# l646773422/h264-lab

Measured on AMD Instinct MI355X. Metric: 1080p macroblocks/sec, higher is better.
Workload: dtype u8

## Files before the change

h264-lab_amd/csrc/enc_mb.h:

```cpp
#ifndef H264E_ENC_MB_H
#define H264E_ENC_MB_H

#include <stddef.h>
#include "enc_kernels.h"

struct GCtx { mv32 mv_left[4], mv_tl[4], mv_top[8]; };
#define GSCR_OFF(t) ((t) == 0 ? 0 : (t) == 1 ? 1024 : (t) == 2 ? 1536 : 2048)
#define GSCR_BYTES 2304

struct MbBuf
{
    alignas(16) uint8_t inp[256];
    alignas(16) uint8_t inp_c[128];
    alignas(16) uint8_t pred[256];
    alignas(4) uint8_t pix_top[36];
    alignas(4) uint8_t ptop[96];
    mv32 mv_top[8];
    uint8_t nnz_top[8];
    int8_t i4_top[4];
    uint32_t df_nz_top;
    int top_type, top_qp;
    mv32 mv[16], mvd[16];
    int type, cost, used_cand;
    mv32 mv_skip_pred;
// ... 309 lines not shown
                    const uint32_t q00 = IP(mv), q02 = IP(v02), q20 = IP(v20), q22 = IP(v22);
#undef IP
                    probe(r, q00, q02, q20, q22);
                }
            }
            sv[0] = (int)t0; sv[1] = (int)t1; sv[2] = (int)t2; sv[3] = (int)t3; sv[4] = (int)t4; sv[5] = (int)t5; sv[6] = (int)t6;
        }, s8);
        wave_sync();
        int best = -1, c8[8];
        mv32 vbest = mv;
        {
            const int pax = hp_pq_vertical, p_step = pax ? mvy(pq) : mvx(pq), s_step = pax ? mvx(sq) : mvy(sq);
            const int p_mv = pax ? mvy(mv) : mvx(mv), s_mv = pax ? mvx(mv) : mvy(mv), p_pr = pax ? mvy(mv_pred) : mvx(mv_pred), s_pr = pax ? mvx(mv_pred) : mvy(mv_pred);
            int P[4], S[4];
            grp_eval4([&](int k) -> int { return se_len((int16_t)(p_mv + k*p_step) - p_pr); }, P);
            grp_eval4([&](int k) -> int { return se_len((int16_t)(s_mv + k*s_step) - s_pr); }, S);
            c8[0] = MUL_LAMBDA(P[2] + S[0], m.lambda_mv); c8[1] = MUL_LAMBDA(P[1] + S[0], m.lambda_mv); c8[2] = MUL_LAMBDA(P[0] + S[2], m.lambda_mv);
            c8[3] = MUL_LAMBDA(P[0] + S[1], m.lambda_mv); c8[4] = MUL_LAMBDA(P[1] + S[1], m.lambda_mv); c8[5] = MUL_LAMBDA(P[2] + S[2], m.lambda_mv);
            c8[6] = MUL_LAMBDA(P[2] + S[1], m.lambda_mv);
        }
#define TRY(j, vv) { const int cst = s8[j] + c8[j]; if (cst < min_sad) { min_sad = cst; vbest = (vv); best = j; } }
        TRY(0, v02) TRY(1, v01) TRY(2, v20) TRY(3, v10) TRY(4, v11) TRY(5, v22) TRY(6, v12)
#undef TRY
        const int pa = best < 0 ? 0 : best == 0 ? 1 : best == 1 ? 0 : best == 2 ? 2 : best == 3 ? 0 : best == 4 ? 1 : best == 5 ? 3 : 3;
        const int pb = best == 1 ? 1 : best == 3 ? 2 : best == 4 ? 2 : best == 6 ? 1 : pa;
        GRP_FOR(i)
        {
            for (int k = 0; k < npass; k++)
            {
                const int d = i + 16*k, r = d >> (g >> 1), c4 = d & (g - 1), o = w*r + 4*c4;
                const uint32_t x = lds32(scr + pa*plane + o), y = lds32(scr + pb*plane + o);
                lds32_store(dst + 16*r + 4*c4, AVG4(x, y));
            }
        }
#undef AVG4
        wave_sync();
        mv = vbest;
    }
    STAMP(L, 26);
    return min_sad;
}

DEV void search_type(RowLds &L, const MbBuf &B, const MbCtx &m, int t, mv32 mv_best, int sad_best0, const rect_t &lim, int skip_cost)
{
    GCtx &X = L.gctx[t];
    int imv = 0, part_sad = MUL_LAMBDA(t == 0 ? 1 : t == 3 ? 12 : 4, m.lambda_q4);
    const int w = (t & 2) ? 8 : 16, h = (t & 1) ? 8 : 16;
    int px = 0, py = 0;
    uint8_t *test = L.gtest[t], *scr = L.gscr + GSCR_OFF(t);
    for (;;)
    {
        rect_t range;
        mv32 mvabs = mb_abs(m, mv_best);
        int sad_best = sad_best0;
        const mv32 mvp = mvp_get_arr(X.mv_left, X.mv_tl, X.mv_top, m.avail, px >> 2, py >> 2, w >> 2, h >> 2);
        if (!t) set_range(mvabs, range, lim, m.y*64 + py*4);
        else
        {
            mvabs = mvround(mb_abs(m, mvp));
            set_range(mvabs, range, lim, m.y*64 + py*4);
            sad_best = grp_sad_ref(m.rv, px + (mvx(mvabs) >> 2), py + (mvy(mvabs) >> 2), B.inp + 16*py + px, w, h)
                     + mv_cost(m, mvabs, mb_abs(m, mvp));
        }
        STAMP(L, 24);
        part_sad += diamond_g(L, B, m, px, py, mvabs, range, mb_abs(m, mvp), sad_best, w, h, test + 16*py + px, scr);
        const mv32 mv = mvsub(mvabs, mvmk(m.x*64, m.y*64));
        L.part_mvd[t][imv] = mvsub(mv, mvp);
        L.part_mv[t][imv++] = mv;
        mvp_put_arr(X.mv_left, X.mv_tl, X.mv_top, px >> 2, py >> 2, w >> 2, h >> 2, mv);
        wave_sync();
        STAMP(L, 27);
        if (t == 0) L.early_bound = imax(part_sad, skip_cost);
        px = (px + w) & 15;
        if (!px)
        {
            py = (py + h) & 15;
            if (!py) break;
        }
    }
    L.gcost[t] = part_sad;
    L.gnum[t] = imv;
}

DEV void partition_hints(const int sad[4], int mode[4])
{
    int sum = sad[0] + sad[1] + sad[2] + sad[3];
    int slope = iabs((sad[0] - sad[2]) + (sad[1] - sad[3])) - iabs((sad[0] - sad[1]) + (sad[2] - sad[3]));
    int skew = iabs(sad[3] - sad[0]) - iabs(sad[2] - sad[1]);
    if (slope > (sum >> 4)) mode[1] = 1;
    if (slope < -(sum >> 4)) mode[2] = 1;
    if (iabs(skew) > (sum >> 4) && iabs(slope) <= (sum >> 4)) mode[3] = 1;
}

DEV void predict_chroma_inter(const MbBuf &B, const MbCtx &m, uint8_t *pred_c)
{
    int w = (m.type & 2) ? 4 : 8, h = (m.type & 1) ? 4 : 8, part = 0, x = 0, y = 0;
    if (m.type == -1) w = h = 8;
    for (;; part++)
    {
        wave_interp_chroma(m.rv, m.ref[1], m.ref[2], x, y, mb_abs(m, B.mv[part]), w, h, pred_c + 16*y + x);
        x = (x + w) & 7;
        if (!x)
        {
            y = (y + h) & 7;
            if (!y) break;
        }
    }
}

DEV int skip_chroma_ok(const MbBuf &B, const MbCtx &m, const uint8_t *pred_c)
{
    const int thr = m.skip_thr;
    for (int c = 0; c < 2; c++)
    {
        int sad = wave_sum([&](int l) -> int {
            if (l >= 16) return 0;
            int r = l >> 1, g = l & 1;
            uint32_t a = lds32(B.inp_c + 16*r + 8*c + 4*g);
            uint32_t p = (m.cropped && r < 4) ? lds32(B.inp_c + 16*(2*r + c) + 8*c + 4*g) : lds32(pred_c + 16*r + 8*c + 4*g);
            return (int)sad4_u8(a, p, 0);
        });
        if (sad >= thr) return 0;
    }
    return 1;
}

template <class SIG> DEV void inter_choose(RowLds &L, MbBuf &B, MbCtx &m, SIG sig)
{
    int prefer[4] = { 1, 0, 0, 0 };
    const RefView &R = m.rv;
    const int bx = m.x*16, by = m.y*16;
    int sad, sad_skip = 0x7FFFFFFF, sad_best = 0x7FFFFFFF, cand_cost_best = 0, j = 0, ncand = 0, sad4[4];
    mv32 mv_best = MV_NA;
    LaneArr cand;
    cand.clear();

    const mv32 mv_pred16 = mvp_get(L, B, m, 0, 0, 4, 4);
    m.mv_skip_pred = 0;
    if (!(~m.avail & (AV_L | AV_T)) && L.mv_left[0] != 0 && B.mv_top[0] != 0) m.mv_skip_pred = mv_pred16;
    const mv32 mv_skip = m.mv_skip_pred, mv_skip_a = mb_abs(m, mv_skip);

    STAMP(L, 2);
    if (in_rect(mv_skip_a, mv_qlimit(m)))
    {
        wave_interp_luma(R, 0, 0, mv_skip_a, 16, 16, L.skip_pred);
        sad_skip = wave_sad_lds_q(B.inp, L.skip_pred, sad4);
        if (imax(imax(sad4[0], sad4[1]), imax(sad4[2], sad4[3])) < m.skip_thr)
        {
            m.type = -1;
            B.mv[0] = mv_skip;
            m.cost = 0;
            predict_chroma_inter(B, m, L.skip_pred_c);
            if (skip_chroma_ok(B, m, L.skip_pred_c))
            {
                wave_copy_wh(B.pred, L.skip_pred, 16, 16);
                return;
            }
        }
        if (m.speed < 1) partition_hints(sad4, prefer);
        mv_best = mvround(mv_skip);
        cand.set(ncand++, mv_best);
        if (!((mvx(mv_skip) | mvy(mv_skip)) & 3))
        {
            sad_best = sad_skip;
            cand_cost_best = mv_cost(m, mv_skip, mv_pred16);
            j = 1;
// ... 453 lines not shown
```

h264-lab_amd/csrc/enc_selftest.h:

```cpp
#ifndef H264E_ENC_SELFTEST_H
#define H264E_ENC_SELFTEST_H
#include "enc_row.h"

struct StageLds
{
    alignas(16) uint8_t win[WIN_W*WIN_STRIDE + 16];
    alignas(16) uint8_t a[256], b[256], o[256];
    alignas(16) qblk_t q[16];
    alignas(4) int16_t dc[16], lev[16], coef[16];
    alignas(4) uint16_t qdat[42];
    CavlcTab ct;
    I4Scratch i4s;
    DfTab df;
    alignas(16) uint8_t yt[20*YT_STRIDE];
    alignas(16) uint8_t ctile[2][10*CT_STRIDE];
    alignas(4) uint8_t bs[32];
    alignas(4) uint8_t nb[5*24];
};
#define STAGE_IN_MAX (96*96 + 256)
#define STAGE_NARGS 24
#define STAGE_OUT_MAX (16 + 16*64 + 32 + 32 + 256)
DEV void stage_selftest(StageLds &S, RowLds &L, int stage, const GLOBAL_AS uint8_t *in, const int *args, GLOBAL_AS uint8_t *out)
{
    int a[STAGE_NARGS];
// ... 40 lines not shown
            if (l < 8) { lds32_store((uint8_t *)S.dc + 4*l, 0u); lds32_store((uint8_t *)S.lev + 4*l, 0u); }
            for (int k = l; k < 256; k += 64) lds32_store((uint8_t *)S.q + 4*k, 0u);
        }
        wave_sync();
        unsigned nz = 0;
        int dcflag = 0;
        WAVE_FOR(l) { lds32_store(S.o + 4*l, lds32(S.b + 4*l)); }
        wave_sync();
        if (mode == QMODE_INTER) nz = wave_xform_quant_recon<QMODE_INTER>(S.a, S.b, S.o, 16, S.q, S.dc, S.lev, S.qdat, (int *)0);
        else if (mode == QMODE_I16) nz = wave_xform_quant_recon<QMODE_I16>(S.a, S.b, S.o, 16, S.q, S.dc, S.lev, S.qdat, (int *)0);
        else if (mode == QMODE_CHROMA) nz = wave_xform_quant_recon<QMODE_CHROMA>(S.a, S.b, S.o, 16, S.q, S.dc, S.lev, S.qdat, &dcflag);
        else nz = i4_block_code(i4q_make(S.qdat), S.a, S.b, S.o, 16, S.q);
        wave_sync();
        WAVE_FOR(l)
        {
            for (int k = l; k < 256; k += 64) gstore32((gu8 *)out + 8 + 4*k, lds32((const uint8_t *)S.q + 4*k));
            if (l < 8) { gstore32((gu8 *)out + 8 + 1024 + 4*l, lds32((const uint8_t *)S.dc + 4*l)); gstore32((gu8 *)out + 8 + 1056 + 4*l, lds32((const uint8_t *)S.lev + 4*l)); }
        }
        wave_sync();
        WAVE_FOR(l) { gstore32((gu8 *)out + 8 + 1088 + 4*l, lds32(S.o + 4*l)); }
        if (wave_lane() == 0) { oi[0] = (int32_t)nz; oi[1] = dcflag; }
        (void)side;
    } else if (stage == 5)
    {
        cavlc_tab_load(S.ct);
        WAVE_FOR(l) { if (l < 8) lds32_store((uint8_t *)S.coef + 4*l, gload32((const gu8 *)in + 4*l)); }
        wave_sync();
        BitW b;
        b.acc = 0; b.nacc = 0; b.pos = 0; b.cap = 60; b.overflow = 0; b.buf = (GLOBAL_AS uint32_t *)(out + 8);
        const int nnz = cavlc_block(b, S.ct, S.coef, a[0], a[1], a[2]);
        const uint32_t nbits = bw_bits(b);
        if (b.nacc) bw_put(b, 32 - b.nacc, 0);
        if (wave_lane() == 0) { oi[0] = nnz; oi[1] = (int32_t)nbits; }
    } else if (stage == 6)
    {
        WAVE_FOR(l)
        {
            if (l < 13)
            {
                const uint8_t e = in[l];
                if (l < 4) S.nb[24*(4 - l) + 3] = e;
                else S.nb[3 + (l - 4)] = e;
            }
            if (l < 16) lds32_store(S.a + 4*l, gload32((const gu8 *)in + 16 + 4*l));
            if (l < 16) lds32_store(S.o + 4*l, 0u);
        }
        wave_sync();
        const int res = wave_i4_choose(S.a, S.o, a[0], S.nb + 24 + 4, a[1], a[2], S.i4s, i4_lanes_make(24));
        wave_sync();
        WAVE_FOR(l) { if (l < 16) gstore32((gu8 *)out + 8 + 4*l, lds32(S.o + 4*l)); }
        if (wave_lane() == 0) { oi[0] = res & 15; oi[1] = res >> 4; }
    } else if (stage == 7)
    {
        const int ny = 20*YT_STRIDE, nc = 10*CT_STRIDE;
        df_tab_load(S.df);
        WAVE_FOR(l)
        {
            for (int k = l; k < ny; k += 64) S.yt[k] = in[k];
            for (int k = l; k < nc; k += 64) { S.ctile[0][k] = in[ny + k]; S.ctile[1][k] = in[ny + nc + k]; }
            if (l < 32) S.bs[l] = in[ny + 2*nc + l];
        }
        wave_sync();
        wave_deblock(S.yt, S.ctile[0], S.ctile[1], S.bs, a[0], a[1], a[2], S.df);
        wave_sync();
        WAVE_FOR(l)
        {
            for (int k = l; k < ny; k += 64) out[k] = S.yt[k];
            for (int k = l; k < nc; k += 64) { out[ny + k] = S.ctile[0][k]; out[ny + nc + k] = S.ctile[1][k]; }
        }
    } else if (stage == 8)
    {
        h264e_geom_t Gs;
        MbCtx m;
        Plane P8 = { (const gu8 *)in, 96, 96, 96 };
        Gs.width = Gs.W = 96; Gs.height = Gs.H = 96; Gs.nmbx = Gs.nmby = 6; Gs.nmb = 36; Gs.cropping = 0;
        Gs.lim_x0 = a[15]; Gs.lim_y0 = a[16]; Gs.lim_x1 = a[17]; Gs.lim_y1 = a[18];
        m.G = &Gs; m.speed = a[10]; m.slice_type = 0; m.x = 2; m.y = 2; m.num = 14; m.qp = a[9];
        m.lambda_mv = k_lambda_mv_q4[a[9]];
        m.rv = R; m.rv.P = P8; m.rv.nmbx = 6; m.rv.nmby = 6;
        if (a[19]) { m.rv.has_win = 1; m.rv.win = (const lu8 *)L.win; m.rv.wx0 = 32 - WIN_M; m.rv.wy0 = 32 - WIN_M; wave_load_window(L.win, P8, m.rv.wx0, m.rv.wy0, 0); }
        WAVE_FOR(l) { lds32_store(L.mb[0].inp + 4*l, gload32((const gu8 *)in + 96*96 + 4*l)); lds32_store(L.gtest[0] + 4*l, 0u); }
        wave_sync();
        const rect_t range = { a[11], a[12], a[13], a[14] };
        GRP_EACH(grp)
        {
            if (grp == (a[20] & 3))
            {
                mv32 mv = mvmk(a[4], a[5]);
                const int cost = diamond_g(L, L.mb[0], m, a[0], a[1], mv, range, mvmk(a[6], a[7]), a[8], a[2], a[3], L.gtest[0] + 16*a[1] + a[0], L.gscr);
                L.gcost[0] = cost; L.gcost[1] = mvx(mv); L.gcost[2] = mvy(mv);
            }
        }
        wave_sync();
        WAVE_FOR(l) { gstore32((gu8 *)out + 16 + 4*l, lds32(L.gtest[0] + 4*l)); }
        if (wave_lane() == 0) { oi[0] = L.gcost[0]; oi[1] = L.gcost[1]; oi[2] = L.gcost[2]; }
    }
}

DEV uint32_t sv_h32(uint32_t a)
{
    a ^= a >> 16; a *= 0x7feb352du; a ^= a >> 15; a *= 0x846ca68bu; a ^= a >> 16;
    return a;
}
DEV int sv_lattice(int32_t ix, int32_t iy, uint32_t seed) { return (int)(sv_h32((uint32_t)ix*0x9E3779B1u ^ (uint32_t)iy*0x85EBCA77u ^ seed) & 255); }
DEV int sv_tex(int32_t X, int32_t Y, uint32_t seed, int lg)
{
    int32_t c = 1 << lg, ix = X >> lg, iy = Y >> lg, fx = X & (c - 1), fy = Y & (c - 1);
    int32_t a = sv_lattice(ix, iy, seed), b = sv_lattice(ix + 1, iy, seed), cc = sv_lattice(ix, iy + 1, seed), d = sv_lattice(ix + 1, iy + 1, seed);
    int32_t top = a*(c - fx) + b*fx, bot = cc*(c - fx) + d*fx;
    return (top*(c - fy) + bot*fy + (1 << (2*lg - 1))) >> (2*lg);
}
DEV uint8_t sv_sample(int w, int h, int t, uint32_t seed, int idx)
{
    const int32_t OFF = 1 << 20;
    if (idx < w*h)
    {
        int x = idx % w, y = idx / w, fw = w/8 > 32 ? w/8 : 32, fh = h/6 > 32 ? h/6 : 32;
        int fx0 = (w/2 + ((10*t) >> 2)) % (w - fw), fy0 = h/3, v;
        if (x >= fx0 && x < fx0 + fw && y >= fy0 && y < fy0 + fh) v = sv_tex(4*x - 10*t + OFF, 4*y + OFF, seed + 1, 5);
        else v = (sv_tex(4*x + 5*t + OFF, 4*y + 3*t + OFF, seed, 6)*3 >> 2) + 32;
        v += (int)(sv_h32((uint32_t)x ^ ((uint32_t)y << 12) ^ ((uint32_t)t << 24) ^ (uint32_t)(seed*7919u)) % 5) - 2;
        return (uint8_t)clip255(v);
    }
    idx -= w*h;
    const int cw = w/2, ch = h/2, pl = idx >= cw*ch;
    if (pl) idx -= cw*ch;
    int x = idx % cw, y = idx / cw;
    if (!pl) return (uint8_t)(128 + ((sv_tex(8*x + 5*t + OFF, 8*y + 3*t + OFF, seed + 2, 7) - 128) >> 2));
    return (uint8_t)(128 - ((sv_tex(8*x + 5*t + OFF, 8*y + 3*t + OFF, seed + 3, 7) - 128) >> 3));
}

#endif
```

h264-lab_amd/csrc/h264e_kernels.hip:

```cpp
#include <stdio.h>
#include <stdlib.h>
#include <string.h>
#include "enc_row.h"
#include "enc_selftest.h"
#include "../../include/h264e_hip.h"

#include <hip/hip_runtime.h>





#ifndef H264E_POLL_SLEEP
#define H264E_POLL_SLEEP 16
#endif
DEV int poll_progress(const GLOBAL_AS int *flag, int need, int &seen, unsigned spin_limit)
{
    unsigned spins = 0;
    for (;;)
    {
        seen = uni(__hip_atomic_load(flag, __ATOMIC_RELAXED, __HIP_MEMORY_SCOPE_AGENT));
        if (seen >= need) return 0;
        if (seen < 0) return seen;
        if (++spins > spin_limit) return -1;
// ... 300 lines not shown
                }
                seen_dep = lowest;
                if (!st) consumer_acquire();
            }
            STAMP(L, 13);
            if (WAVES >= 2 && !st && x >= 2) st = lds_wait(&L.f_wdone, x - 1, &L.f_stop);
            STAMP(L, 23);
            if (!st) row_prefetch<GEOM>(L, G, RT, row, x);
            STAMP(L, 0);
            if (uni(abort_v) == launch_id) st = -2;
            if (!st && seen < need)
            {
                seen = uni(early);
                if (seen < 0) st = seen;
                else if (seen < need) st = poll_progress(above, need, seen, G.spin_limit);
                if (!st) consumer_acquire();
            }
            STAMP(L, 13);
            if (!st) load_top<WAVES >= 2 ? LOAD_TOP_MV : LOAD_TOP_ALL>(L, L.mb[x & 1], G, C.bottom + (size_t)(row - 1)*G.nmbx, C.pend + (size_t)(row - 1)*G.nmbx, x, row > row0);
            STAMP(L, 0);
            if (WAVES >= 2 && !st && x >= 1) st = lds_wait(&L.f_decided, x, &L.f_stop);
            STAMP(L, 6);
            if (st)
            {
                if (WAVES >= 2) { flag_set(&L.f_stop, st); return; }
                if (LANE == 0)
                {
                    if (st == -1) *errflag = 1;
                    __hip_atomic_store(my_progress, st, __ATOMIC_RELAXED, __HIP_MEMORY_SCOPE_AGENT);
                }
                count_mbs(x);
                return;
            }
            if (WAVES == 1) row_step<GEOM>(L, G, C, RT, row, x, row0, row1);
            else mb_search<GEOM>(L, L.mb[x & 1], G, RT, row, x, row0, SearchSignals{ &L, x + 1, WAVES >= 3 });
            if (WAVES >= 3 && uni(flag_get(&L.f_stop))) return;
            {
                const int ff = uni(L.far_fail[0]) | (WAVES == 1 ? uni(L.far_fail[1]) : 0);
                if (ff)
                {
                    if (WAVES >= 2) { flag_set(&L.f_stop, ff < -2 ? -2 : ff); return; }
                    if (LANE == 0)
                    {
                        if (ff == -1) *errflag = 1;
                        __hip_atomic_store(my_progress, ff < -2 ? -2 : ff, __ATOMIC_RELAXED, __HIP_MEMORY_SCOPE_AGENT);
                    }
                    count_mbs(x);
                    return;
                }
            }
            if (WAVES >= 2) { flag_set(&L.f_inter, x + 1); STAMP(L, 14); continue; }
            asm volatile("s_waitcnt vmcnt(0)" ::: "memory");
            __builtin_amdgcn_wave_barrier();
            publish(my_progress, x + 1);
            STAMP(L, 14);
        }
        if (WAVES >= 2)
        {
#ifdef H264E_STAMPS
            if (LANE < 32 && C.prof) atomicAdd(C.prof + LANE, L.prof[0][LANE]);
#endif
            return;
        }
    } else if (WAVES >= 3 && wv == 2)
    {
        for (int x = 0; x < G.nmbx; x++)
        {
            int req = 0, st = 0;
            for (unsigned spins = 0;; spins++)
            {
                const int r3 = uni(flag_get(&L.f_t3req));
                if (r3 == x + 1) { req = 1; break; }
                if (r3 > x + 1) break;
                if (uni(flag_get(&L.f_inter)) >= x + 1) break;
                if (uni(flag_get(&L.f_stop))) { st = 1; break; }
                if (spins > LDS_SPIN_LIMIT) { flag_set(&L.f_stop, -1); st = 1; break; }
                __builtin_amdgcn_s_sleep(H264E_LDS_SLEEP);
            }
            if (st) return;
            if (!req) continue;
            MbCtx m;
            mb_ctx_init<GEOM>(m, L, G, RT, row, x, row0, 2);
            const rect_t lim = { uni(L.t3_lim[0]), uni(L.t3_lim[1]), uni(L.t3_lim[2]), uni(L.t3_lim[3]) };
            const mv32 mv_best = (mv32)uni(L.t3_mv_best);
            const int sad_best = uni(L.t3_sad_best);
            GRP_EACH(t)
            {
                if (t == 3) search_type(L, L.mb[x & 1], m, 3, mv_best, sad_best, lim, 0);
            }
            wave_sync();
            const int ff = uni(L.far_fail[2]);
            if (ff) { flag_set(&L.f_stop, ff < -2 ? -2 : ff); return; }
            flag_set(&L.f_t3done, x + 1);
        }
#ifdef H264E_STAMPS
        if (LANE < 32 && C.prof) atomicAdd(C.prof + LANE, L.prof[2][LANE]);
#endif
        return;
    } else if (WAVES == 4 && wv == 3)
    {
        for (int x = 0; x < G.nmbx; x++)
        {
            const int st = lds_wait(&L.f_front, x + 1, &L.f_stop);
            if (st)
            {
                if (LANE == 0) __hip_atomic_store(my_progress, st == -2 ? -2 : -1, __ATOMIC_RELAXED, __HIP_MEMORY_SCOPE_AGENT);
                return;
            }
            MbCtx m;
            mb_ctx_init<GEOM>(m, L, G, RT, row, x, row0, 1);
            m.type = uni(L.d_type[x & 1]);
            mb_recon_back<GEOM>(L, L.mb[x & 1], m, G, C, RT, row, x, row0, row1);
            asm volatile("s_waitcnt vmcnt(0)" ::: "memory");
            __builtin_amdgcn_wave_barrier();
            publish(my_progress, x + 1);
            flag_set(&L.f_wdone, x + 1);
        }
#ifdef H264E_STAMPS
        if (LANE < 32 && C.prof) atomicAdd(C.prof + LANE, L.prof[3][LANE]);
#endif
        return;
    } else
    {
        GLOBAL_AS int *my_decided = my_progress + G.nmby;
        GLOBAL_AS h264e_mbbottom_t *rowrec = C.bottom + (size_t)row*G.nmbx;
        int seen = 0;
        for (int x = 0; x < G.nmbx; x++)
        {
            MbBuf &B = L.mb[x & 1];
            MbCtx m;
            mb_ctx_init<GEOM>(m, L, G, RT, row, x, row0, 1);
            int ff = 0;
            const int need = row > row0 ? imin(x + 2, G.nmbx) : 0;
            if (seen < need)
            {
                ff = poll_progress(C.progress + (row - 1), need, seen, G.spin_limit);
                if (!ff) consumer_acquire();
                else flag_set(&L.f_stop, ff);
            }
            STAMP(L, 17);
            if (!ff)
            {
                load_top<LOAD_TOP_REST>(L, B, G, C.bottom + (size_t)(row - 1)*G.nmbx, C.pend + (size_t)(row - 1)*G.nmbx, x, row > row0);
                if (!mb_intra_decide(L, B, m, RT, InterFromSearchWave{ &L, x + 1, WAVES == 4 })) ff = uni(flag_get(&L.f_stop));
                else
                {
                    flag_set(&L.f_decided, x + 1);
                    WAVE_FOR(l) { if (l < 4) cstore32((gu8 *)(rowrec + x) + 32 + 4*l, (uint32_t)B.mv_top[l]); }
                    const auto publish_decided = [&]() {
                        asm volatile("s_waitcnt vmcnt(0)" ::: "memory");
                        __builtin_amdgcn_wave_barrier();
                        publish(my_decided, x + 1);
                    };
                    if (WAVES == 4)
                    {
                        mb_recon_front<GEOM>(L, B, m, G, C, RT, row, x, row0, row1, publish_decided);
                        L.d_type[x & 1] = m.type;
                    } else mb_recon_write<GEOM>(L, B, m, G, C, RT, row, x, row0, row1, publish_decided);
                    ff = uni(L.far_fail[1]);
                    if (ff) { ff = ff < -2 ? -2 : ff; flag_set(&L.f_stop, ff); }
                    else if (WAVES == 4) flag_set(&L.f_front, x + 1);
                }
            }
            if (ff)
            {
                if (LANE == 0)
                {
                    if (ff == -1) *errflag = 1;
                    __hip_atomic_store(my_decided, ff, __ATOMIC_RELAXED, __HIP_MEMORY_SCOPE_AGENT);
                    if (WAVES != 4) __hip_atomic_store(my_progress, ff, __ATOMIC_RELAXED, __HIP_MEMORY_SCOPE_AGENT);
                }
                count_mbs(x);
                return;
// ... 101 lines not shown
```

h264-lab_amd/csrc/wave.h:

```cpp
#ifndef H264E_WAVE_H
#define H264E_WAVE_H

#include <stdint.h>
#include <string.h>

#ifdef H264E_EMU
extern "C" void emu_check_global(const void *p, size_t n, const char *file, int line);
#define EMU_GLOBAL(p, n) emu_check_global((const void *)(p), (n), __FILE__, __LINE__)
#define GLOBAL_AS
#define LDS_AS
#define NOINLINE_DEV static __attribute__((noinline))
#define DEV static inline
#define DEVM inline
#define DCONST static const
#ifdef H264E_EMU_REVERSE
#define WAVE_FOR(l) for (int l = 63; l >= 0; --l)
#else
#define WAVE_FOR(l) for (int l = 0; l < 64; ++l)
#endif
struct u32x4 { uint32_t x, y, z, w; };
DEV void wave_sync() {}
DEV int wave_lane() { return 0; }
DEV int uni(int v) { return v; }
template <class F> DEV int wave_sum(F f)
{
    int s = 0;
    for (int l = 0; l < 64; ++l) s += f(l);
    return s;
}
template <class F> DEV void wave_sum4(F f, int out[4])
{
    out[0] = out[1] = out[2] = out[3] = 0;
    for (int l = 0; l < 64; ++l)
    {
        int v[4] = { 0, 0, 0, 0 };
        f(l, v);
        for (int k = 0; k < 4; ++k) out[k] += v[k];
    }
}
template <class F> DEV void wave_sum8(F f, int out[8])
{
    for (int k = 0; k < 8; ++k) out[k] = 0;
    for (int l = 0; l < 64; ++l)
    {
        int v[8] = { 0, 0, 0, 0, 0, 0, 0, 0 };
        f(l, v);
        for (int k = 0; k < 8; ++k) out[k] += v[k];
    }
}
template <class F> DEV uint64_t wave_ballot(F f)
{
    uint64_t m = 0;
    for (int l = 0; l < 64; ++l) if (f(l)) m |= 1ull << l;
    return m;
}
DEV uint32_t sad4_u8(uint32_t a, uint32_t b, uint32_t acc)
{
    for (int k = 0; k < 4; ++k)
    {
        int d = (int)((a >> (8*k)) & 255) - (int)((b >> (8*k)) & 255);
        acc += (uint32_t)(d < 0 ? -d : d);
    }
    return acc;
}
DEV int clz32(uint32_t v) { return __builtin_clz(v); }
DEV uint32_t bswap32(uint32_t v) { return __builtin_bswap32(v); }

#define GRP_EACH(g) for (int g = 0; g < 4; ++g)
#ifdef H264E_EMU_REVERSE
#define GRP_FOR(i) for (int i = 15; i >= 0; --i)
#else
#define GRP_FOR(i) for (int i = 0; i < 16; ++i)
#endif
template <class F> DEV int grp_sum(F f)
{
    int s = 0;
    for (int i = 0; i < 16; ++i) s += f(i);
    return s;
}
template <class F> DEV void grp_sum4(F f, int out[4])
{
    out[0] = out[1] = out[2] = out[3] = 0;
    for (int i = 0; i < 16; ++i)
    {
        int v[4] = { 0, 0, 0, 0 };
        f(i, v);
        for (int k = 0; k < 4; ++k) out[k] += v[k];
    }
}
template <class F> DEV void grp_sum8(F f, int out[8])
{
    for (int k = 0; k < 8; ++k) out[k] = 0;
    for (int i = 0; i < 16; ++i)
    {
        int v[8] = { 0, 0, 0, 0, 0, 0, 0, 0 };
        f(i, v);
        for (int k = 0; k < 8; ++k) out[k] += v[k];
    }
}
template <class F> DEV void grp_eval4(F f, int out[4]) { for (int d = 0; d < 4; ++d) out[d] = f(d); }
template <class F> DEV void grp_eval8(F f, int out[8]) { for (int d = 0; d < 8; ++d) out[d] = f(d); }
DEV void grp_count(int *p) { *p += 1; }

struct V16 { int v[16]; };
#define V16_BINOP(op) DEV V16 operator op(const V16 &a, const V16 &b) { V16 r; for (int i = 0; i < 16; i++) r.v[i] = a.v[i] op b.v[i]; return r; }
V16_BINOP(+) V16_BINOP(-) V16_BINOP(*) V16_BINOP(&) V16_BINOP(|)
#undef V16_BINOP
DEV V16 operator>>(const V16 &a, int s) { V16 r; for (int i = 0; i < 16; i++) r.v[i] = a.v[i] >> s; return r; }
DEV V16 v16_splat(int s) { V16 r; for (int i = 0; i < 16; i++) r.v[i] = s; return r; }
template <class F> DEV V16 v16_make(F f) { V16 r; for (int i = 0; i < 16; i++) r.v[i] = f(i, 0); return r; }
template <class F> DEV V16 v16_map(const V16 &a, F f) { V16 r; for (int i = 0; i < 16; i++) r.v[i] = f(i, a.v[i]); return r; }
template <class F> DEV V16 v16_map2(const V16 &a, const V16 &b, F f) { V16 r; for (int i = 0; i < 16; i++) r.v[i] = f(i, a.v[i], b.v[i]); return r; }
template <class F> DEV V16 v16_map3(const V16 &a, const V16 &b, const V16 &c, F f) { V16 r; for (int i = 0; i < 16; i++) r.v[i] = f(i, a.v[i], b.v[i], c.v[i]); return r; }
template <class F> DEV void v16_each(const V16 &a, F f) { for (int i = 0; i < 16; i++) f(i, 0, a.v[i]); }
DEV int v16_any(const V16 &a) { for (int i = 0; i < 16; i++) if (a.v[i]) return 1; return 0; }
DEV V16 v16_tile_any(const V16 &a) { V16 r; const int n = v16_any(a); for (int i = 0; i < 16; i++) r.v[i] = n; return r; }
DEV unsigned v16_tiles_nonzero(const V16 &a) { return (unsigned)v16_any(a); }
struct V16C { };
DEV V16C v16c_make() { return V16C(); }
template <class F> DEV V16 v16_make(const V16C &, F f) { return v16_make(f); }
template <class F> DEV V16 v16_map(const V16C &, const V16 &a, F f) { return v16_map(a, f); }
template <class F> DEV V16 v16_map2(const V16C &, const V16 &a, const V16 &b, F f) { return v16_map2(a, b, f); }
template <class F> DEV V16 v16_map3(const V16C &, const V16 &a, const V16 &b, const V16 &c, F f) { return v16_map3(a, b, c, f); }
template <class F> DEV void v16_each(const V16C &, const V16 &a, F f) { v16_each(a, f); }
DEV V16 v16_tile_any(const V16C &, const V16 &a) { return v16_tile_any(a); }
template <class V> DEV V v16_fwd4x4_c(const V16C &, const V &d) { return v16_fwd4x4(d); }
template <class V> DEV V v16_inv4x4_c(const V16C &, const V &c) { return v16_inv4x4(c); }
template <int P0, int P1, int P2, int P3> DEV V16 v16_quadperm(const V16 &a)
{
    const int p[4] = { P0, P1, P2, P3 };
    V16 r;
    for (int i = 0; i < 16; i++) r.v[i] = a.v[(i & ~3) | p[i & 3]];
    return r;
}
DEV V16 v16_xpose(const V16 &a) { V16 r; for (int i = 0; i < 16; i++) r.v[i] = a.v[(i & 3)*4 + (i >> 2)]; return r; }
DEV V16 v16_from(const V16 &a, const V16 &idx) { V16 r; for (int i = 0; i < 16; i++) r.v[i] = a.v[idx.v[i] & 15]; return r; }
DEV unsigned v16_nonzero_mask(const V16 &a) { unsigned m = 0; for (int i = 0; i < 16; i++) if (a.v[i]) m |= 1u << i; return m; }
#define V16_TILES 1

template <class P> DEV P uniptr(P p) { return p; }
DEV uint32_t alignbyte32(uint32_t hi, uint32_t lo, unsigned sh) { return (uint32_t)((((uint64_t)hi << 32) | lo) >> (8*(sh & 3))); }
DEV uint32_t ld32_aligned(const void *q) { uint32_t v; memcpy(&v, q, 4); return v; }
DEV int opaque_int(int v) { return v; }
DEV int mul24(int a, int b) { return a*b; }
DEV int popc32(uint32_t v) { return __builtin_popcount(v); }
DEV int dep_poll(const int *p) { EMU_GLOBAL(p, 4); return 0x7fffffff; }
DEV void wave_nap() {}
DEV void consumer_acquire() {}
DEV void drain_stores() {}
DEV void g_atomic_add(int *p, int v) { EMU_GLOBAL(p, 4); *p += v; }
DEV int g_atomic_load(const int *p) { EMU_GLOBAL(p, 4); return *p; }
DEV void g_atomic_store(int *p, int v) { EMU_GLOBAL(p, 4); *p = v; }
struct V64 { int v[64]; };
template <class F> DEV V64 v64_make(F f) { V64 r; WAVE_FOR(l) r.v[l] = f(l); return r; }
template <class F> DEV V64 v64_map(const V64 &a, F f) { V64 r; WAVE_FOR(l) r.v[l] = f(l, a.v[l]); return r; }
template <class F> DEV void v64_each(const V64 &a, F f) { WAVE_FOR(l) f(l, a.v[l]); }
DEV V64 v64_quad_sum(const V64 &a) { V64 r; for (int l = 0; l < 64; l++) r.v[l] = a.v[l & ~3] + a.v[(l & ~3) + 1] + a.v[(l & ~3) + 2] + a.v[(l & ~3) + 3]; return r; }
DEV int v64_read(const V64 &a, int lane) { return a.v[lane]; }
DEV int v64_own(const V64 &a, int lane) { return a.v[lane]; }
template <class F> DEV void v64_each3(const V64 &a, const V64 &b, const V64 &c, F f) { WAVE_FOR(l) f(l, a.v[l], b.v[l], c.v[l]); }
DEV V64 v64_row_shr1(const V64 &a) { V64 r; for (int l = 0; l < 64; l++) r.v[l] = (l & 15) ? a.v[l - 1] : a.v[l]; return r; }
DEV V64 v64_row_shl1(const V64 &a) { V64 r; for (int l = 0; l < 64; l++) r.v[l] = (l & 15) != 15 ? a.v[l + 1] : a.v[l]; return r; }
DEV V64 v64_row_quadmin(const V64 &a)
{
    V64 r;
    for (int l = 0; l < 64; l++) { int m = a.v[l]; for (int q = 0; q < 4; q++) { const int v = a.v[(l & 48) | (4*q) | (l & 3)]; if (v < m) m = v; } r.v[l] = m; }
    return r;
}
DEV uint64_t v64_nonzero_ballot(const V64 &a) { uint64_t m = 0; for (int l = 0; l < 64; l++) if (a.v[l]) m |= 1ull << l; return m; }
#define PROF_ROW_BEGIN(L) do { } while (0)
#define PROF_ROW_SYNC(L) do { } while (0)
#define PROF_ROW_END(L, C) do { } while (0)

#else

#include <hip/hip_runtime.h>
#define EMU_GLOBAL(p, n) do { } while (0)
static __device__ __forceinline__ int imin_raw(int a, int b) { return a < b ? a : b; }
static __device__ __forceinline__ int lane_opaque() { int l = (int)(threadIdx.x & 63u); asm volatile("" : "+v"(l)); return l; }
#define LANE lane_opaque()
#define GLOBAL_AS __attribute__((address_space(1)))
#define LDS_AS __attribute__((address_space(3)))
#define NOINLINE_DEV static __device__ __noinline__
#define DEV static __device__ __forceinline__
#define DEVM __device__ __forceinline__
#define DCONST static __device__ const
#define WAVE_FOR(l) for (int l = LANE, _w1 = 1; _w1; _w1 = 0)
typedef uint32_t u32x4 __attribute__((ext_vector_type(4), aligned(4)));
DEV void wave_sync()
{
    __builtin_amdgcn_fence(__ATOMIC_ACQ_REL, "wavefront");
    __builtin_amdgcn_wave_barrier();
}
DEV int wave_lane() { return LANE; }
DEV int uni(int v) { return __builtin_amdgcn_readfirstlane(v); }
DEV int wave_reduce_add(int v)
{
    v += __builtin_amdgcn_update_dpp(0, v, 0xB1, 0xf, 0xf, true);
    v += __builtin_amdgcn_update_dpp(0, v, 0x4E, 0xf, 0xf, true);
    v += __builtin_amdgcn_update_dpp(0, v, 0x141, 0xf, 0xf, true);
    v += __builtin_amdgcn_update_dpp(0, v, 0x140, 0xf, 0xf, true);
    return __builtin_amdgcn_readlane(v, 0) + __builtin_amdgcn_readlane(v, 16) +
           __builtin_amdgcn_readlane(v, 32) + __builtin_amdgcn_readlane(v, 48);
}
template <class F> DEV int wave_sum(F f) { return wave_reduce_add(f(LANE)); }
template <class F> DEV void wave_sum4(F f, int out[4])
{
    int v[4] = { 0, 0, 0, 0 };
    f(LANE, v);
    int a = v[0] | (v[1] << 16), b = v[2] | (v[3] << 16);
    a = wave_reduce_add(a);
    b = wave_reduce_add(b);
    out[0] = a & 0xffff; out[1] = (int)((unsigned)a >> 16);
    out[2] = b & 0xffff; out[3] = (int)((unsigned)b >> 16);
}
template <class F> DEV void wave_sum8(F f, int out[8])
{
    int v[8] = { 0, 0, 0, 0, 0, 0, 0, 0 };
    f(LANE, v);
#pragma unroll
    for (int k = 0; k < 4; k++)
    {
        int a = wave_reduce_add(v[2*k] | (v[2*k + 1] << 16));
        out[2*k] = a & 0xffff; out[2*k + 1] = (int)((unsigned)a >> 16);
    }
}
template <class F> DEV uint64_t wave_ballot(F f) { return __ballot(f(LANE)); }
DEV uint32_t sad4_u8(uint32_t a, uint32_t b, uint32_t acc) { return __builtin_amdgcn_sad_u8(a, b, acc); }
DEV int clz32(uint32_t v) { return __clz((int)v); }
DEV uint32_t bswap32(uint32_t v) { return __builtin_bswap32(v); }

#define GRP_EACH(g) for (int g = LANE >> 4, _e1 = 1; _e1; _e1 = 0)
#define GRP_FOR(i) for (int i = LANE & 15, _g1 = 1; _g1; _g1 = 0)
DEV int row_reduce_add(int v)
{
    v += __builtin_amdgcn_update_dpp(0, v, 0xB1, 0xf, 0xf, true);
    v += __builtin_amdgcn_update_dpp(0, v, 0x4E, 0xf, 0xf, true);
    v += __builtin_amdgcn_update_dpp(0, v, 0x141, 0xf, 0xf, true);
    v += __builtin_amdgcn_update_dpp(0, v, 0x140, 0xf, 0xf, true);
    return v;
}
template <class F> DEV int grp_sum(F f) { return row_reduce_add(f(LANE & 15)); }
template <class F> DEV void grp_sum4(F f, int out[4])
{
    int v[4] = { 0, 0, 0, 0 };
    f(LANE & 15, v);
    const int a = row_reduce_add(v[0] | (v[1] << 16)), b = row_reduce_add(v[2] | (v[3] << 16));
    out[0] = a & 0xffff; out[1] = (int)((unsigned)a >> 16);
    out[2] = b & 0xffff; out[3] = (int)((unsigned)b >> 16);
}
template <class F> DEV void grp_sum8(F f, int out[8])
{
    int v[8] = { 0, 0, 0, 0, 0, 0, 0, 0 };
    f(LANE & 15, v);
#pragma unroll
    for (int k = 0; k < 4; k++)
    {
        const int a = row_reduce_add(v[2*k] | (v[2*k + 1] << 16));
        out[2*k] = a & 0xffff; out[2*k + 1] = (int)((unsigned)a >> 16);
    }
}
template <class F> DEV void grp_eval4(F f, int out[4])
{
    const int c = f(LANE & 3);
    out[0] = __builtin_amdgcn_update_dpp(0, c, 0x00, 0xf, 0xf, true); out[1] = __builtin_amdgcn_update_dpp(0, c, 0x55, 0xf, 0xf, true);
    out[2] = __builtin_amdgcn_update_dpp(0, c, 0xAA, 0xf, 0xf, true); out[3] = __builtin_amdgcn_update_dpp(0, c, 0xFF, 0xf, 0xf, true);
}
template <class F> DEV void grp_eval8(F f, int out[8])
{
    const int c0 = f(LANE & 3), c1 = f(4 + (LANE & 3));
    out[0] = __builtin_amdgcn_update_dpp(0, c0, 0x00, 0xf, 0xf, true); out[1] = __builtin_amdgcn_update_dpp(0, c0, 0x55, 0xf, 0xf, true);
    out[2] = __builtin_amdgcn_update_dpp(0, c0, 0xAA, 0xf, 0xf, true); out[3] = __builtin_amdgcn_update_dpp(0, c0, 0xFF, 0xf, 0xf, true);
    out[4] = __builtin_amdgcn_update_dpp(0, c1, 0x00, 0xf, 0xf, true); out[5] = __builtin_amdgcn_update_dpp(0, c1, 0x55, 0xf, 0xf, true);
    out[6] = __builtin_amdgcn_update_dpp(0, c1, 0xAA, 0xf, 0xf, true); out[7] = __builtin_amdgcn_update_dpp(0, c1, 0xFF, 0xf, 0xf, true);
}
DEV void grp_count(int *p) { if ((LANE & 15) == 0) __hip_atomic_fetch_add(p, 1, __ATOMIC_RELAXED, __HIP_MEMORY_SCOPE_WORKGROUP); }

struct V16 { int v; };
#define V16_BINOP(op) DEV V16 operator op(const V16 &a, const V16 &b) { V16 r; r.v = a.v op b.v; return r; }
V16_BINOP(+) V16_BINOP(-) V16_BINOP(*) V16_BINOP(&) V16_BINOP(|)
#undef V16_BINOP
DEV V16 operator>>(const V16 &a, int s) { V16 r; r.v = a.v >> s; return r; }
DEV V16 v16_splat(int s) { V16 r; r.v = s; return r; }
template <class F> DEV V16 v16_make(F f) { V16 r; r.v = f(LANE & 15, LANE >> 4); return r; }
template <class F> DEV V16 v16_map(const V16 &a, F f) { V16 r; r.v = f(LANE & 15, a.v); return r; }
template <class F> DEV V16 v16_map2(const V16 &a, const V16 &b, F f) { V16 r; r.v = f(LANE & 15, a.v, b.v); return r; }
template <class F> DEV V16 v16_map3(const V16 &a, const V16 &b, const V16 &c, F f) { V16 r; r.v = f(LANE & 15, a.v, b.v, c.v); return r; }
template <class F> DEV void v16_each(const V16 &a, F f) { f(LANE & 15, LANE >> 4, a.v); }
DEV int v16_any(const V16 &a) { return __ballot(a.v != 0) != 0; }
DEV V16 v16_tile_any(const V16 &a)
{
    const unsigned long long m = __ballot(a.v != 0);
    const int t = LANE >> 4;
    const unsigned w = (t & 2) ? (unsigned)(m >> 32) : (unsigned)m;
    V16 r;
    r.v = ((w >> (16*(t & 1))) & 0xffffu) != 0;
    return r;
}
DEV unsigned v16_tiles_nonzero(const V16 &a)
{
    const unsigned long long m = __ballot(a.v != 0);
    const unsigned lo = (unsigned)m, hi = (unsigned)(m >> 32);
    return ((lo & 0xffffu) ? 1u : 0u) | ((lo >> 16) ? 2u : 0u) | ((hi & 0xffffu) ? 4u : 0u) | ((hi >> 16) ? 8u : 0u);
}
template <int P0, int P1, int P2, int P3> DEV V16 v16_quadperm(const V16 &a)
{
    V16 r;
    r.v = __builtin_amdgcn_update_dpp(0, a.v, P0 | (P1 << 2) | (P2 << 4) | (P3 << 6), 0xf, 0xf, true);
    return r;
}
DEV V16 v16_xpose(const V16 &a)
{
    V16 r;
    r.v = __builtin_amdgcn_ds_bpermute(4*((LANE & 48) | ((LANE & 3) << 2) | ((LANE >> 2) & 3)), a.v);
    return r;
}
DEV V16 v16_from(const V16 &a, const V16 &idx)
{
    V16 r;
    r.v = __builtin_amdgcn_ds_bpermute(4*((LANE & 48) | (idx.v & 15)), a.v);
    return r;
}
struct V16C
{
    int i, tile;
    int xp;
    int f_s, f_ka, f_kb;
    int i_sh, i_a1, i_a2, i_s;
};
DEV V16C v16c_make()
{
    V16C c;
    const int l = LANE, x = l & 3;
    c.i = l & 15; c.tile = l >> 4;
    c.xp = 4*((l & 48) | ((l & 3) << 2) | ((l >> 2) & 3));
    c.f_s = (x & 2) ? -1 : 1;
    c.f_ka = x == 1 ? 2 : 1; c.f_kb = x == 0 ? 1 : x == 1 ? 1 : x == 2 ? -1 : -2;
    c.i_sh = x & 1; c.i_a1 = x == 2 ? -1 : 1; c.i_a2 = x == 1 ? -1 : 1; c.i_s = (x & 2) ? -1 : 1;
    return c;
}
template <class F> DEV V16 v16_make(const V16C &c, F f) { V16 r; r.v = f(c.i, c.tile); return r; }
template <class F> DEV V16 v16_map(const V16C &c, const V16 &a, F f) { V16 r; r.v = f(c.i, a.v); return r; }
template <class F> DEV V16 v16_map2(const V16C &c, const V16 &a, const V16 &b, F f) { V16 r; r.v = f(c.i, a.v, b.v); return r; }
template <class F> DEV V16 v16_map3(const V16C &c, const V16 &a, const V16 &b, const V16 &d, F f) { V16 r; r.v = f(c.i, a.v, b.v, d.v); return r; }
// ... 170 lines not shown
```

Baseline: 13.70 million.

## Run 8x8 partition search on whole wave with four diamond directions in parallel

Replaces the type-3 (8x8) search on the dedicated wave, which previously ran only in one 16-lane group via GRP_EACH, with a new whole-wave diamond search. Each 16-lane row evaluates one of the four diamond neighbours at once, and a new wave_grp_sums helper reduces them. Subpel refinement is done across all 64 lanes with a fused 6-tap interpolation and eight candidate SADs. The aim is to use the idle lanes and cut the serial latency of the 8x8 search. The risk is that search decisions differ slightly from the grouped path, and the added code may increase register pressure.

Measured after the change: 13.70 million, median of 4. Within noise of the previous version (+0.0%).

```diff
diff --git a/h264-lab_amd/csrc/enc_mb.h b/h264-lab_amd/csrc/enc_mb.h
--- a/h264-lab_amd/csrc/enc_mb.h
+++ b/h264-lab_amd/csrc/enc_mb.h
@@ -415,6 +415,208 @@
     L.gnum[t] = imv;
 }
 
+DEV int diamond_w8(RowLds &L, const MbBuf &B, const MbCtx &m, int px, int py, mv32 &mv_io, const rect_t &range, mv32 mv_pred, int min_sad, uint8_t *dst)
+{
+    const RefView &R = m.rv;
+    const uint8_t *b = B.inp + 16*py + px;
+    mv32 mv = (mv32)uni(mv_io);
+    min_sad = uni(min_sad);
+    int c0, c1, c2, c3, p0, p1, p2, p3;
+#define DX(d) ((d) == 0 ? 4 : (d) == 1 ? -4 : 0)
+#define DY(d) ((d) == 2 ? 4 : (d) == 3 ? -4 : 0)
+#define SEL4(d, a0, a1, a2, a3) ((d) == 0 ? (a0) : (d) == 1 ? (a1) : (d) == 2 ? (a2) : (a3))
+    for (;;)
+    {
+        int d0 = 0, dir_prev = -1;
+        c0 = c1 = c2 = c3 = p0 = p1 = p2 = p3 = 0xffff;
+        for (;;)
+        {
+            const int e0 = mvx(mv) + 4 <= range.x1 && c0 == 0xffff, e1 = mvx(mv) - 4 >= range.x0 && c1 == 0xffff;
+            const int e2 = mvy(mv) + 4 <= range.y1 && c2 == 0xffff, e3 = mvy(mv) - 4 >= range.y0 && c3 == 0xffff;
+            if (!(e0 | e1 | e2 | e3)) break;
+            const int want = e0 | (e1 << 1) | (e2 << 2) | (e3 << 3);
+            int b4[4];
+            const int cx = px + (mvx(mv) >> 2), cy = py + (mvy(mv) >> 2);
+            const auto cost_of = [&](int d, int i) -> int { return i == 0 ? mv_cost(m, mvadd(mv, mvmk(DX(d), DY(d))), mv_pred) : 0; };
+            if (rv_inside(R, cx - 1, cy - 1, cx + 8, cy + 8))
+            {
+                const lu8 *base = rv_ptr(R, cx, cy);
+                wave_grp_sums([&](int l) -> int {
+                    const int d = l >> 4, i = l & 15, r = i >> 1, c4 = i & 1;
+                    const int off = d == 0 ? 1 : d == 1 ? -1 : d == 2 ? WIN_STRIDE : -WIN_STRIDE;
+                    return (int)sad4_u8(lds32u(base + r*WIN_STRIDE + 4*c4 + off), lds32(b + 16*r + 4*c4), 0) + cost_of(d, i);
+                }, b4);
+            } else
+            {
+                rv_wait_rect(R, cy - 1, cx + 8, cy + 8);
+                wave_grp_sums([&](int l) -> int {
+                    const int d = l >> 4, i = l & 15, r = i >> 1, c4 = i & 1;
+                    uint32_t s = 0;
+                    if ((want >> d) & 1) s = sad4_u8(ref_load4(R.P, cx + 4*c4 + (DX(d) >> 2), cy + r + (DY(d) >> 2)), lds32(b + 16*r + 4*c4), 0);
+                    return (int)s + cost_of(d, i);
+                }, b4);
+            }
+            const int b0 = b4[0], b1 = b4[1], b2 = b4[2], b3 = b4[3];
+            const int o0 = (0 - d0) & 3, o1 = (1 - d0) & 3, o2 = (2 - d0) & 3, o3 = (3 - d0) & 3;
+            const int wk = imin(imin((e0 && b0 < min_sad) ? o0 : 4, (e1 && b1 < min_sad) ? o1 : 4), imin((e2 && b2 < min_sad) ? o2 : 4, (e3 && b3 < min_sad) ? o3 : 4));
+            const int lim = wk < 4 ? wk : 3;
+            if (e0 && o0 <= lim) c0 = b0 & 0xffff;
+            if (e1 && o1 <= lim) c1 = b1 & 0xffff;
+            if (e2 && o2 <= lim) c2 = b2 & 0xffff;
+            if (e3 && o3 <= lim) c3 = b3 & 0xffff;
+            if (wk == 4) break;
+            {
+                const int win = (d0 + wk) & 3;
+                const int corner = dir_prev >= 0 ? SEL4(win, p0, p1, p2, p3) : 0xffff;
+                const int back = win ^ 1, side = dir_prev >= 0 ? (dir_prev ^ 1) : -1;
+                p0 = c0; p1 = c1; p2 = c2; p3 = c3;
+                c0 = back == 0 ? (min_sad & 0xffff) : side == 0 ? corner : 0xffff;
+                c1 = back == 1 ? (min_sad & 0xffff) : side == 1 ? corner : 0xffff;
+                c2 = back == 2 ? (min_sad & 0xffff) : side == 2 ? corner : 0xffff;
+                c3 = back == 3 ? (min_sad & 0xffff) : side == 3 ? corner : 0xffff;
+                min_sad = SEL4(win, b0, b1, b2, b3);
+                mv = mvadd(mv, mvmk(DX(win), DY(win)));
+                dir_prev = win;
+                d0 = win;
+            }
+        }
+
+        const int pri = c3 >= c2 ? 2 : 3, sec = c1 >= c0 ? 0 : 1;
+        const mv32 v = mvadd(mv, mvmk(DX(pri) + DX(sec), DY(pri) + DY(sec)));
+        if (in_rect(v, range))
+        {
+            const int cost = wave_sad_ref(R, px + (mvx(v) >> 2), py + (mvy(v) >> 2), b, 8, 8) + mv_cost(m, v, mv_pred);
+            if (cost < min_sad)
+            {
+                mv = v;
+                min_sad = cost;
+                continue;
+            }
+        }
+        break;
+    }
+    STAMP(L, 25);
+#undef SEL4
+#undef DX
+#undef DY
+
+#ifdef H264E_ABLATE
+    if (H264E_ABLATE == 3) { wave_interp_luma(R, px, py, mv, 8, 8, dst); mv_io = mv; return min_sad; }
+#endif
+    if (!(m.speed < 9 && in_rect(mv, mv_qlimit(m))))
+    {
+        wave_interp_luma(R, px, py, mv, 8, 8, dst);
+        mv_io = mv;
+        return min_sad;
+    }
+    {
+        mv32 pq = mvmk(0, -1), sq = mvmk(-1, 0);
+        uint32_t ms1 = c1, ms2 = c3;
+        if (c3 >= c2) { pq = mvmk(0, 1); ms2 = c2; }
+        if (c1 >= c0) { sq = mvmk(1, 0); ms1 = c0; }
+        if (ms2 > ms1) { mv32 sw = sq; sq = pq; pq = sw; }
+        const mv32 vdg = mvadd(pq, sq);
+        const mv32 v02 = mvadd(mv, mvadd(pq, pq)), v01 = mvadd(mv, pq), v20 = mvadd(mv, mvadd(sq, sq)), v10 = mvadd(mv, sq);
+        const mv32 v11 = mvadd(mv, vdg), v22 = mvadd(mv, mvadd(vdg, vdg)), v12 = mvadd(mv, mvadd(pq, vdg));
+        const int fx0 = px + (mvx(mv) >> 2), fy0 = py + (mvy(mv) >> 2);
+        const bool inside = rv_inside(R, fx0 - 5, fy0 - 3, fx0 + 8 + 4, fy0 + 8 + 3);
+        if (!inside) rv_wait_rect(R, fy0 - 3, fx0 + 8 + 4, fy0 + 8 + 3);
+        const int hp_ox = mvx(vdg) < 0 ? 1 : 0, hp_oy = mvy(vdg) < 0 ? 1 : 0, hp_pq_vertical = mvx(pq) == 0;
+        const V64 Q = v64_make([&](int l) -> int {
+            const int ix = fx0 + (l & 7) - hp_ox, iy = fy0 + (l >> 3) - hp_oy;
+            int th[6], cb[6];
+#pragma unroll
+            for (int j = 0; j < 6; j++)
+            {
+                uint32_t lo, hi;
+                if (inside)
+                {
+                    const lu8 *q = rv_ptr(R, ix - 2, iy - 2 + j);
+                    const unsigned sh = (unsigned)(uintptr_t)q & 3;
+                    const LDS_AS uint32_t *w = (const LDS_AS uint32_t *)(q - sh);
+                    const uint32_t d0 = ld32_aligned(w), d1 = ld32_aligned(w + 1), d2 = ld32_aligned(w + 2);
+                    lo = alignbyte32(d1, d0, sh); hi = alignbyte32(d2, d1, sh);
+                } else
+                {
+                    lo = ref_load4(R.P, ix - 2, iy - 2 + j); hi = ref_load4(R.P, ix + 2, iy - 2 + j);
+                }
+                const int a0 = (int)(lo & 255), a1 = (int)((lo >> 8) & 255), a2 = (int)((lo >> 16) & 255), a3 = (int)(lo >> 24);
+                th[j] = tap6(a0, a1, a2, a3, (int)(hi & 255), (int)((hi >> 8) & 255));
+                cb[j] = hp_ox ? a3 : a2;
+            }
+            const int fh = clip255(shr_opaque((hp_oy ? th[3] : th[2]) + 16, 5));
+            const int fv = clip255(shr_opaque(tap6(cb[0], cb[1], cb[2], cb[3], cb[4], cb[5]) + 16, 5));
+            const int fd = clip255(shr_opaque(tap6w(th[0], th[1], th[2], th[3], th[4], th[5]) + 512, 10));
+            const int full = hp_oy ? cb[3] : cb[2];
+            return full | ((hp_pq_vertical ? fv : fh) << 8) | ((hp_pq_vertical ? fh : fv) << 16) | (fd << 24);
+        });
+#define AVG4(x, y) (((x) | (y)) - ((((x) ^ (y)) >> 1) & 0x7f7f7f7fu))
+        int s8[8];
+        wave_sum8([&](int l, int *sv) {
+            const uint32_t q = (uint32_t)v64_own(Q, l), in = b[16*(l >> 3) + (l & 7)];
+            const uint32_t q00 = q & 255, q02 = (q >> 8) & 255, q20 = (q >> 16) & 255, q22 = q >> 24;
+            const uint32_t q01 = AVG4(q00, q02), q10 = AVG4(q00, q20), q11 = AVG4(q02, q20), q12 = AVG4(q22, q02);
+            sv[0] = (int)sad4_u8(q02, in, 0); sv[1] = (int)sad4_u8(q01, in, 0); sv[2] = (int)sad4_u8(q20, in, 0);
+            sv[3] = (int)sad4_u8(q10, in, 0); sv[4] = (int)sad4_u8(q11, in, 0); sv[5] = (int)sad4_u8(q22, in, 0);
+            sv[6] = (int)sad4_u8(q12, in, 0);
+        }, s8);
+        int best = -1, c8[8];
+        mv32 vbest = mv;
+        {
+            const int pax = hp_pq_vertical, p_step = pax ? mvy(pq) : mvx(pq), s_step = pax ? mvx(sq) : mvy(sq);
+            const int p_mv = pax ? mvy(mv) : mvx(mv), s_mv = pax ? mvx(mv) : mvy(mv), p_pr = pax ? mvy(mv_pred) : mvx(mv_pred), s_pr = pax ? mvx(mv_pred) : mvy(mv_pred);
+            int P[3], S[3];
+#pragma unroll
+            for (int k = 0; k < 3; k++) { P[k] = se_len((int16_t)(p_mv + k*p_step) - p_pr); S[k] = se_len((int16_t)(s_mv + k*s_step) - s_pr); }
+            c8[0] = MUL_LAMBDA(P[2] + S[0], m.lambda_mv); c8[1] = MUL_LAMBDA(P[1] + S[0], m.lambda_mv); c8[2] = MUL_LAMBDA(P[0] + S[2], m.lambda_mv);
+            c8[3] = MUL_LAMBDA(P[0] + S[1], m.lambda_mv); c8[4] = MUL_LAMBDA(P[1] + S[1], m.lambda_mv); c8[5] = MUL_LAMBDA(P[2] + S[2], m.lambda_mv);
+            c8[6] = MUL_LAMBDA(P[2] + S[1], m.lambda_mv);
+        }
+#define TRY(j, vv) { const int cst = s8[j] + c8[j]; if (cst < min_sad) { min_sad = cst; vbest = (vv); best = j; } }
+        TRY(0, v02) TRY(1, v01) TRY(2, v20) TRY(3, v10) TRY(4, v11) TRY(5, v22) TRY(6, v12)
+#undef TRY
+        const int pa = best < 0 ? 0 : best == 0 ? 1 : best == 1 ? 0 : best == 2 ? 2 : best == 3 ? 0 : best == 4 ? 1 : 3;
+        const int pb = best == 1 ? 1 : best == 3 ? 2 : best == 4 ? 2 : best == 6 ? 1 : pa;
+        v64_each(Q, [&](int l, int q) {
+            const uint32_t x = ((uint32_t)q >> (8*pa)) & 255, y = ((uint32_t)q >> (8*pb)) & 255;
+            dst[16*(l >> 3) + (l & 7)] = (uint8_t)AVG4(x, y);
+        });
+#undef AVG4
+        wave_sync();
+        mv = vbest;
+    }
+    STAMP(L, 26);
+    mv_io = mv;
+    return min_sad;
+}
+
+DEV void search_8x8_w(RowLds &L, const MbBuf &B, const MbCtx &m, const rect_t &lim)
+{
+    GCtx &X = L.gctx[3];
+    int part_sad = MUL_LAMBDA(12, m.lambda_q4);
+    for (int k = 0; k < 4; k++)
+    {
+        const int px = 8*(k & 1), py = 8*(k >> 1);
+        rect_t range;
+        const mv32 mvp = (mv32)uni(mvp_get_arr(X.mv_left, X.mv_tl, X.mv_top, m.avail, px >> 2, py >> 2, 2, 2));
+        const mv32 pred = mb_abs(m, mvp);
+        mv32 mvabs = mvround(pred);
+        set_range(mvabs, range, lim, m.y*64 + py*4);
+        const int sad_best = wave_sad_ref(m.rv, px + (mvx(mvabs) >> 2), py + (mvy(mvabs) >> 2), B.inp + 16*py + px, 8, 8) + mv_cost(m, mvabs, pred);
+        STAMP(L, 24);
+        part_sad += diamond_w8(L, B, m, px, py, mvabs, range, pred, sad_best, L.gtest[3] + 16*py + px);
+        const mv32 mv = mvsub(mvabs, mvmk(m.x*64, m.y*64));
+        L.part_mvd[3][k] = mvsub(mv, mvp);
+        L.part_mv[3][k] = mv;
+        mvp_put_arr(X.mv_left, X.mv_tl, X.mv_top, px >> 2, py >> 2, 2, 2, mv);
+        wave_sync();
+        STAMP(L, 27);
+    }
+    L.gcost[3] = part_sad;
+    L.gnum[3] = 4;
+    wave_sync();
+}
+
 DEV void partition_hints(const int sad[4], int mode[4])
 {
     int sum = sad[0] + sad[1] + sad[2] + sad[3];
diff --git a/h264-lab_amd/csrc/enc_selftest.h b/h264-lab_amd/csrc/enc_selftest.h
--- a/h264-lab_amd/csrc/enc_selftest.h
+++ b/h264-lab_amd/csrc/enc_selftest.h
@@ -146,7 +146,13 @@
         WAVE_FOR(l) { lds32_store(L.mb[0].inp + 4*l, gload32((const gu8 *)in + 96*96 + 4*l)); lds32_store(L.gtest[0] + 4*l, 0u); }
         wave_sync();
         const rect_t range = { a[11], a[12], a[13], a[14] };
-        GRP_EACH(grp)
+        if (a[20] == 4)
+        {
+            mv32 mv = mvmk(a[4], a[5]);
+            const int cost = diamond_w8(L, L.mb[0], m, a[0], a[1], mv, range, mvmk(a[6], a[7]), a[8], L.gtest[0] + 16*a[1] + a[0]);
+            L.gcost[0] = cost; L.gcost[1] = mvx(mv); L.gcost[2] = mvy(mv);
+        }
+        else GRP_EACH(grp)
         {
             if (grp == (a[20] & 3))
             {
diff --git a/h264-lab_amd/csrc/h264e_kernels.hip b/h264-lab_amd/csrc/h264e_kernels.hip
--- a/h264-lab_amd/csrc/h264e_kernels.hip
+++ b/h264-lab_amd/csrc/h264e_kernels.hip
@@ -406,13 +406,7 @@
             MbCtx m;
             mb_ctx_init<GEOM>(m, L, G, RT, row, x, row0, 2);
             const rect_t lim = { uni(L.t3_lim[0]), uni(L.t3_lim[1]), uni(L.t3_lim[2]), uni(L.t3_lim[3]) };
-            const mv32 mv_best = (mv32)uni(L.t3_mv_best);
-            const int sad_best = uni(L.t3_sad_best);
-            GRP_EACH(t)
-            {
-                if (t == 3) search_type(L, L.mb[x & 1], m, 3, mv_best, sad_best, lim, 0);
-            }
-            wave_sync();
+            search_8x8_w(L, L.mb[x & 1], m, lim);
             const int ff = uni(L.far_fail[2]);
             if (ff) { flag_set(&L.f_stop, ff < -2 ? -2 : ff); return; }
             flag_set(&L.f_t3done, x + 1);
diff --git a/h264-lab_amd/csrc/wave.h b/h264-lab_amd/csrc/wave.h
--- a/h264-lab_amd/csrc/wave.h
+++ b/h264-lab_amd/csrc/wave.h
@@ -97,6 +97,11 @@
         f(i, v);
         for (int k = 0; k < 8; ++k) out[k] += v[k];
     }
+}
+template <class F> DEV void wave_grp_sums(F f, int out[4])
+{
+    out[0] = out[1] = out[2] = out[3] = 0;
+    for (int l = 0; l < 64; ++l) out[l >> 4] += f(l);
 }
 template <class F> DEV void grp_eval4(F f, int out[4]) { for (int d = 0; d < 4; ++d) out[d] = f(d); }
 template <class F> DEV void grp_eval8(F f, int out[8]) { for (int d = 0; d < 8; ++d) out[d] = f(d); }
@@ -260,6 +265,12 @@
         out[2*k] = a & 0xffff; out[2*k + 1] = (int)((unsigned)a >> 16);
     }
 }
+template <class F> DEV void wave_grp_sums(F f, int out[4])
+{
+    const int v = row_reduce_add(f(LANE));
+    out[0] = __builtin_amdgcn_readlane(v, 0); out[1] = __builtin_amdgcn_readlane(v, 16);
+    out[2] = __builtin_amdgcn_readlane(v, 32); out[3] = __builtin_amdgcn_readlane(v, 48);
+}
 template <class F> DEV void grp_eval4(F f, int out[4])
 {
     const int c = f(LANE & 3);
```
